# GitHubOfAndrew/TeAMOFlow

Hardware: AMD Instinct MI355X
Metric: train_interactions_per_sec (higher is better)
Workload: dtype f32

## Files before the change

include/tmf.h:

```cpp
#ifndef TMF_H
#define TMF_H

#include <stddef.h>
#include <stdint.h>

#ifdef __cplusplus
extern "C" {
#endif

#define TMF_VERSION 203

#define TMF_OK 0
#define TMF_E_INVALID (-1)
#define TMF_E_LAUNCH (-2)
#define TMF_E_UNSUPPORTED (-3)

#define TMF_EPI_ADAM 0
#define TMF_EPI_GRAD 1

int tmf_version(void);
const char* tmf_last_error(void);

int tmf_padded_ld(int n_components);

// ... 94 lines not shown
                         int n_components, void* stream);
int tmf_wmrb_scores3_bf16(const tmf_slice_lists* lists, const void* U, const void* V, float* sp, float* p,
                          int n_components, void* stream);
int tmf_wmrb_scores5_users_per_workgroup(void);
int tmf_wmrb_scores5_supported(int n_components, int bf16, int64_t n_items);
size_t tmf_wmrb_scores5_workspace_bytes(int64_t n_wg, int32_t n_windows, int wgs_per_launch);
int tmf_wmrb_scores5_f32(const int32_t* ids, const int32_t* outs, const int64_t* wg_ptr, int64_t n_wg, int64_t n_users,
                         int64_t n_items, const void* U, const void* V, float* sp, float* p, int n_components,
                         int wgs_per_launch, const int32_t* wstart, int32_t n_windows, int lag, void* workspace,
                         size_t workspace_bytes, void* stream);
int tmf_wmrb_scores5_bf16(const int32_t* ids, const int32_t* outs, const int64_t* wg_ptr, int64_t n_wg, int64_t n_users,
                          int64_t n_items, const void* U, const void* V, float* sp, float* p, int n_components,
                          int wgs_per_launch, const int32_t* wstart, int32_t n_windows, int lag, void* workspace,
                          size_t workspace_bytes, void* stream);
int tmf_wmrb_scores6_users_per_group(void);
int tmf_wmrb_scores6_supported(int n_components, int bf16, int64_t n_items);
int tmf_wmrb_scores6_f32(const int32_t* ids, const int32_t* outs, const int64_t* chunk_ptr, int64_t n_groups, int32_t n_slices,
                         int64_t n_users, int64_t n_items, const void* U, const void* V, float* sp, float* p, int n_components,
                         void* stream);
int tmf_wmrb_scores6_bf16(const int32_t* ids, const int32_t* outs, const int64_t* chunk_ptr, int64_t n_groups, int32_t n_slices,
                          int64_t n_users, int64_t n_items, const void* U, const void* V, float* sp, float* p, int n_components,
                          void* stream);
int tmf_wmrb_scores7_users_per_group(void);
int tmf_wmrb_scores7_slots(void);
int tmf_wmrb_scores7_supported(int n_components, int bf16, int64_t n_items);
int tmf_wmrb_scores7_f32(const void* steps, const int32_t* place, const int64_t* sub_step, const int64_t* sub_place,
                         const int32_t* chunk_sub, int64_t n_groups, int32_t n_slices, int64_t n_users, int64_t n_items,
                         const void* U, const void* V, float* sp, float* p, int n_components, void* stream);
int tmf_wmrb_hinge2(const int64_t* rowptr, const float* val, const float* p, const float* sp, int32_t n_users,
                    int32_t n_samples, float c, float* delta, float* D, float* loss_part, void* stream);
int tmf_wmrb_hinge2_ordered(const int64_t* rowptr, const float* val, const float* p, const float* sp, int32_t n_users,
                            int32_t n_samples, float c, float* delta, float* D, float* loss_part, const int32_t* user_order,
                            void* stream);
int tmf_bpr_pairs(const int64_t* rowptr, const float* val, const float* p, const float* sp, int32_t n_users, int32_t n_samples,
                  float* delta, float* D, float* loss_part, const int32_t* user_order, void* stream);
int tmf_warp_pairs(const int64_t* rowptr, const float* val, const float* p, const float* sp, int32_t n_users, int32_t n_samples,
                   int32_t n_items, float* delta, float* D, float* loss_part, const int32_t* user_order, void* stream);
int tmf_warp_pairs_ranked(const int64_t* rowptr, const float* val, const float* p, const float* sp, const uint16_t* rank,
                          int32_t n_users, int32_t n_samples, int32_t n_items, float* delta, float* D, float* loss_part,
                          const int32_t* user_order, void* stream);
int tmf_softmax_pairs(const int64_t* rowptr, const float* val, const float* p, const float* sp, int32_t n_users, int32_t n_samples,
                      float c, float* delta, float* D, float* loss_part, const int32_t* user_order, void* stream);
int tmf_wmrb_gradu3_f32(const tmf_slice_lists* lists, const float* D, const float* delta, const void* V, float* part,
                        int per_slice_launches, int n_components, void* stream);
int tmf_wmrb_gradu3_bf16(const tmf_slice_lists* lists, const float* D, const float* delta, const void* V, float* part,
                         int per_slice_launches, int n_components, void* stream);
// ... 194 lines not shown
```

teamoflow_amd/_engine.py:

```python
import ctypes
import os

import torch

from . import _lib

DEFAULT_CHUNK = 1024
PART_BUDGET = int(os.environ.get('TMF_PART_BUDGET', 8 << 30))


def row_bytes(n_components, dtype=torch.float32):
    return _lib.padded_ld(n_components, dtype) * (2 if dtype is torch.bfloat16 else 4)


def _excl_cumsum(x):
    out = torch.zeros(x.numel() + 1, dtype=torch.int64, device=x.device)
    torch.cumsum(x, 0, out=out[1:])
    return out


def take_interactions(indices, values, keep, user_offset=0, item_offset=0):
    u = indices[:, 0][keep] - user_offset
    j = indices[:, 1][keep] - item_offset
    return torch.stack([u, j], dim=1), values[keep]
# ... 486 lines not shown
            self.outs[q0:q0 + q.numel()] = torch.where(r < c, outs_sorted[src], torch.full_like(src, self.PAD).to(i32))
            del q, st, r, c, src
        self.n_entries, self.n_padded = E, E8
        return ptr8, rowptr


class Scores6Plan(_ScoreStreams):

    def __init__(self, plan, wplan, n_components, dtype=torch.float32, slice_bytes=None):
        lib = _lib.load_library()
        self.key = (int(n_components), dtype)
        UG = int(lib.tmf_wmrb_scores6_users_per_group())
        n = plan.n_items
        self.n_groups = ng = -(-wplan.R.shape[0] // UG)
        slice_bytes = int(os.environ.get('TMF_S6_SLICE_BYTES', slice_bytes or SCORES6_SLICE_BYTES))
        ns = int(min(max(1, -(-n * row_bytes(n_components, dtype) // slice_bytes)), max(1, (2 ** 31 - 1) // max(ng, 1))))
        width = -(-n // ns)
        self.n_slices = ns = -(-n // width)
        self.chunk_ptr, _ = self._build(plan, wplan, UG, lambda grp, item: (item // width) * ng + grp, ns * ng)


SCORES7_SLICE_BYTES = 4 << 20
SCORES7_MIN_SHARE = 1.5


def scores7_wanted(plan, wplan, n_components, dtype=torch.float32):
    env = os.environ.get('TMF_SCORES7')
    if env == '0' or wplan is None or not wplan.sliced or not plan.col_u.is_cuda:
        return False
    m, S = wplan.R.shape
    if m * S >= 2 ** 31 or plan.nnz >= 2 ** 31:
        return False
    lib = _lib.load_library()
    if not lib.tmf_wmrb_scores7_supported(int(n_components), int(dtype is torch.bfloat16), int(plan.n_items)):
        return False
    if env == '1':
        return True
    if os.environ.get('TMF_SCORES5') == '1' or os.environ.get('TMF_SCORES6') == '1':
        return False
    if plan.n_items * row_bytes(n_components, dtype) < 8 * VISIT_SLICE_BYTES:
        return False
    UG = int(lib.tmf_wmrb_scores7_users_per_group())
    return UG * (S + plan.nnz / max(m, 1)) / plan.n_items >= SCORES7_MIN_SHARE


class Scores7Plan:

    K = 4

    def __init__(self, plan, wplan, n_components, dtype=torch.float32, slice_bytes=None, slots=None):
        lib = _lib.load_library()
        self.key = (int(n_components), dtype)
        dev, i32, i64, K = plan.col_u.device, torch.int32, torch.int64, self.K
        self.users_per_group = UG = int(lib.tmf_wmrb_scores7_users_per_group())
        self.pad_slot = cap = int(lib.tmf_wmrb_scores7_slots())
        self.slots = SL = max(1, min(cap, int(os.environ.get('TMF_S7_SLOTS', slots or cap))))
        m, S = wplan.R.shape
        n, nnz = plan.n_items, plan.nnz
        E = nnz + m * S
        self.n_groups = ng = -(-m // UG)
        slice_bytes = int(os.environ.get('TMF_S7_SLICE_BYTES', slice_bytes or SCORES7_SLICE_BYTES))
        ns = int(min(max(1, -(-n * row_bytes(n_components, dtype) // slice_bytes)), max(1, (2 ** 31 - 1) // max(ng, 1))))
        self.width = width = -(-n // ns)
        self.n_slices = ns = -(-n // width)
        nc = ns * ng
        ar = torch.arange(E, device=dev, dtype=i64)
# ... 39 lines not shown
        self.sub_step = _excl_cumsum(sub_steps)
        del subA, sub_steps, run_steps
        pos = ar - run_start[run_of]
        del ar, run_start
        stepA = run_step0[run_of] + pos // K
        k = pos % K
        del pos, run_of, run_step0
        users = torch.zeros(n_steps, K, dtype=i64, device=dev)
        slot4 = torch.full((n_steps, K), cap, dtype=i64, device=dev)
        first = k == 0
        users[stepA[first]] = luA[first].to(i64)[:, None]
        users[stepA, k] = luA.to(i64)
        slot4[stepA, k] = slotA.to(i64)
        steps = torch.zeros(n_steps + 1, 4, dtype=i32, device=dev)
        steps[stepA[first], 0] = itemA[first]
        del first, stepA, k, luA, slotA, itemA
        w = users[:, 0] | (users[:, 1] << 8) | (users[:, 2] << 16) | (users[:, 3] << 24)
        steps[:n_steps, 1] = torch.where(w >= 2 ** 31, w - 2 ** 32, w).to(i32)
        steps[:n_steps, 2] = (slot4[:, 0] | (slot4[:, 1] << 16)).to(i32)
        steps[:n_steps, 3] = (slot4[:, 2] | (slot4[:, 3] << 16)).to(i32)
        self.steps = steps
        self.n_entries = E


def scores5_wanted(plan, wplan, n_components, dtype=torch.float32):
    if os.environ.get('TMF_SCORES5') != '1' or wplan is None or not wplan.sliced or not plan.col_u.is_cuda:
        return False
    m, S = wplan.R.shape
    if m * S >= 2 ** 31 or plan.nnz >= 2 ** 31:
        return False
    return bool(_lib.load_library().tmf_wmrb_scores5_supported(int(n_components), int(dtype is torch.bfloat16), int(plan.n_items)))


class Scores5Plan(_ScoreStreams):

    def __init__(self, plan, wplan, n_components, dtype=torch.float32, slice_bytes=None):
        lib = _lib.load_library()
        dev = plan.col_u.device
        self.key = (int(n_components), dtype)
        UB = int(lib.tmf_wmrb_scores5_users_per_workgroup())
        n = plan.n_items
        self.n_wg = n_wg = -(-wplan.R.shape[0] // UB)
        slice_bytes = int(os.environ.get('TMF_S5_SLICE_BYTES', slice_bytes or (512 << 10)))
        ns = int(min(max(1, -(-n * row_bytes(n_components, dtype) // slice_bytes)), 4096, max(1, (2 ** 31 - 1) // max(n_wg, 1))))
        width = -(-n // ns)
        self.n_slices = ns
# ... 78 lines not shown

    def _adopt_wplan(self):
        plan, wplan, dtype, dev = self.plan, self.wplan, self.dtype, self.plan.col_u.device
        need = dict(slab=max(self._slab_fixed,
                             (wplan.seg_e.n_slab if wplan is not None and wplan.seg_e is not None else 0) * self.ld,
                             (wplan.vrows.n_slab if wplan is not None and wplan.vrows is not None else 0) * self.ld))
        self.row_stationary = False
        if wplan is not None and wplan.sliced:
            m, S = wplan.R.shape
            self.row_stationary = row_stationary_wanted(m, plan.n_items, S, plan.nnz, self.r, dtype)
            self.users_per_launch = int(os.environ.get('TMF_G4_USERS', 32768))
            if self.row_stationary:
                nb = _lib.load_library().tmf_wmrb_gradu4_workspace_bytes(m, wplan.n_slices, self.users_per_launch)
                self.g4_sync = torch.zeros(max(nb // 4, 1), dtype=torch.int32, device=dev)
            ns = wplan.n_slices
            if ns * m * self.ld * 4 <= PART_BUDGET:
                self.part_layers, self.gradu_launches = ns, 0
            elif wplan.xcd_major:
                self.part_layers, self.gradu_launches = min(8, ns), 3
            else:
                self.part_layers, self.gradu_launches = 1, 1
            need.update(sp=m * S, pk=max(plan.nnz, 1), part=self.part_layers * max(m, 1) * self.ld)
            if scores7_wanted(plan, wplan, self.r, dtype):
                if wplan.s7 is None or wplan.s7.key != (self.r, dtype):
                    if os.environ.get('TMF_SCORES7') == '1':
                        wplan.s7 = Scores7Plan(plan, wplan, self.r, dtype)
                    else:
                        try:
                            wplan.s7 = Scores7Plan(plan, wplan, self.r, dtype)
                        except torch.OutOfMemoryError:
                            wplan.s7 = None
            else:
                wplan.s7 = None
            if wplan.s7 is None and scores6_wanted(plan, wplan, self.r, dtype):
                if wplan.s6 is None or wplan.s6.key != (self.r, dtype):
                    wplan.s6 = Scores6Plan(plan, wplan, self.r, dtype)
            else:
                wplan.s6 = None
            if wplan.seg_e is not None and scores5_wanted(plan, wplan, self.r, dtype):
                if wplan.s5 is None or wplan.s5.key != (self.r, dtype):
                    wplan.s5 = Scores5Plan(plan, wplan, self.r, dtype)
            else:
                wplan.s5 = None
        if wplan is not None and wplan.rows4:
            L = _lib.load_library()
            per_group = L.tmf_wsum_rows4_rows_per_group(self.r, int(dtype is torch.bfloat16))
            if not per_group:
                raise ValueError('the row-stationary item pass needs rows of at least 16 lanes')
            cus = torch.cuda.get_device_properties(dev).multi_processor_count if torch.cuda.is_available() else 256
            self.rows4_per_launch = int(os.environ.get('TMF_ROWS4_PER_LAUNCH', 2 * cus * per_group))
            n_work = wplan.vrows.n_vrows if wplan.vrows is not None else plan.n_items
            nb = L.tmf_wsum_rows4_workspace_bytes(n_work, wplan.user_chunks, self.rows4_per_launch)
            self.rows4_sync = torch.zeros(max(nb // 4, 1), dtype=torch.int32, device=dev)
        return need
# ... 387 lines not shown

def epoch_logistic(st, adam, loss_out, weighted=False, item_epi=_lib.EPI_ADAM, item_out=None, prof=None, user_epi=_lib.EPI_ADAM,
                   user_out=None):
    _list_passes(st, adam, 'tmf_logistic_pass', 'logistic', st.loss_part, None, (int(bool(weighted)),), loss_out, item_epi, item_out,
                 prof, user_epi, user_out)


def epoch_kl(st, adam, loss_out, item_epi=_lib.EPI_ADAM, item_out=None, prof=None, user_epi=_lib.EPI_ADAM, user_out=None):
    lib, p, r = _lib.get(), st.plan, st.r
    s = _lib.stream_ptr()
    _timed(prof, 'kl_moments', lambda: getattr(lib, 'tmf_kl_moments' + st.sfx)(
        p.seg_u.cstruct(), _lib.ptr(p.col_u), _lib.ptr(p.val_u), _lib.ptr(st.U), _lib.ptr(st.V), _lib.ptr(st.kl_part), r, s))
    _timed(prof, 'kl_coeffs', lambda: lib.tmf_kl_coeffs(_lib.ptr(st.kl_part), p.seg_u.nseg, _lib.ptr(loss_out), _lib.ptr(st.kl_coef), s))
    _list_passes(st, adam, 'tmf_kl_pass', 'kl', st.kl_coef, st.kl_coef, (), None, item_epi, item_out, prof, user_epi, user_out)


def _wmrb_user_pass_sliced(lib, st, adam, c, prof=None, user_epi=_lib.EPI_ADAM, U_out=None, pairs='hinge'):
    p, w, r = st.plan, st.wplan, st.r
    i32 = ctypes.c_int32
    m, S, ns = p.n_users, w.S, w.n_slices
    s = _lib.stream_ptr()
    lists = w.lists(p)
    s5, s6, s7 = w.s5, w.s6, w.s7
    if s7 is not None:
        _timed(prof, 'wmrb_scores', lambda: lib.tmf_wmrb_scores7_f32(
            _lib.ptr(s7.steps), _lib.ptr(s7.place), _lib.ptr(s7.sub_step), _lib.ptr(s7.sub_place), _lib.ptr(s7.chunk_sub), s7.n_groups,
            i32(s7.n_slices), m, p.n_items, _lib.ptr(st.U), _lib.ptr(st.V), _lib.ptr(st.sp), _lib.ptr(st.pk), r, s))
    elif s6 is not None:
        _timed(prof, 'wmrb_scores', lambda: getattr(lib, 'tmf_wmrb_scores6' + st.sfx)(
            _lib.ptr(s6.ids), _lib.ptr(s6.outs), _lib.ptr(s6.chunk_ptr), s6.n_groups, i32(s6.n_slices), m, p.n_items, _lib.ptr(st.U),
            _lib.ptr(st.V), _lib.ptr(st.sp), _lib.ptr(st.pk), r, s))
    elif s5 is not None:
        _timed(prof, 'wmrb_scores', lambda: getattr(lib, 'tmf_wmrb_scores5' + st.sfx)(
            _lib.ptr(s5.ids), _lib.ptr(s5.outs), _lib.ptr(s5.wg_ptr), s5.n_wg, m, p.n_items, _lib.ptr(st.U), _lib.ptr(st.V),
            _lib.ptr(st.sp), _lib.ptr(st.pk), r, s5.wgs_per_launch, _lib.ptr(s5.wstart) if s5.paced else None, i32(s5.n_windows),
            s5.lag, _lib.ptr(s5.sync) if s5.paced else None, s5.sync.numel() * 4, s))
    else:
        _timed(prof, 'wmrb_scores', lambda: getattr(lib, 'tmf_wmrb_scores3' + st.sfx)(lists, _lib.ptr(st.U), _lib.ptr(st.V), _lib.ptr(st.sp),
                                                                                _lib.ptr(st.pk), r, s))
    if pairs == 'bpr':
        _timed(prof, 'bpr_pairs', lambda: lib.tmf_bpr_pairs(_lib.ptr(p.rowptr_u), _lib.ptr(p.val_u), _lib.ptr(st.pk), _lib.ptr(st.sp),
                                                            i32(m), i32(S), _lib.ptr(w.delta), _lib.ptr(w.D), _lib.ptr(st.loss_part),
                                                            _lib.ptr(w.hinge_order), s))
    elif pairs == 'warp':
        rank = w.sample_rank()
        _timed(prof, 'warp_pairs', lambda: lib.tmf_warp_pairs_ranked(_lib.ptr(p.rowptr_u), _lib.ptr(p.val_u), _lib.ptr(st.pk),
                                                                     _lib.ptr(st.sp), _lib.ptr(rank), i32(m), i32(S), i32(p.n_items),
# ... 63 lines not shown
```

teamoflow_amd/_lib.py:

```python
import ctypes
import os
import subprocess

import torch

_HERE = os.path.dirname(os.path.abspath(__file__))
LIB_PATH = os.environ.get('TMF_LIB', os.path.join(_HERE, 'libtmf.so'))
CSRC = os.path.join(_HERE, 'csrc')

EPI_ADAM, EPI_GRAD = 0, 1


class EngineUnavailable(RuntimeError):
    pass


class EngineError(RuntimeError):
    pass


class Adam(ctypes.Structure):
    _fields_ = [('alpha', ctypes.c_float), ('one_minus_b1', ctypes.c_float), ('one_minus_b2', ctypes.c_float),
                ('eps', ctypes.c_float)]

# ... 47 lines not shown
    'tmf_mse_pass_f32': (_I, [_SEG, _P, _P, _P, _P, _P, _P, _P, _I, _I, Adam, _P]),
    'tmf_kl_moments_f32': (_I, [_SEG, _P, _P, _P, _P, _P, _I, _P]),
    'tmf_kl_moments_bf16': (_I, [_SEG, _P, _P, _P, _P, _P, _I, _P]),
    'tmf_kl_coeffs': (_I, [_P, _L, _P, _P, _P]),
    'tmf_kl_pass_f32': (_I, [_SEG, _P, _P, _P, _P, _P, _P, _P, _I, _I, Adam, _P]),
    'tmf_kl_pass_bf16': (_I, [_SEG, _P, _P, _P, _P, _P, _P, _P, _I, _I, Adam, _P]),
    'tmf_logistic_pass_f32': (_I, [_SEG, _P, _P, _P, _P, _P, _P, _P, _I, _I, Adam, _I, _P]),
    'tmf_logistic_pass_bf16': (_I, [_SEG, _P, _P, _P, _P, _P, _P, _P, _I, _I, Adam, _I, _P]),
    'tmf_wsum_pass_f32': (_I, [_SEG, _P, _P, _P, _P, _P, _P, _P, _I, _I, Adam, _P]),
    'tmf_wsum_rows4_rows_per_group': (_I, [_I, _I]),
    'tmf_wsum_rows4_workspace_bytes': (_SZ, [_I32, _I32, _I32]),
    'tmf_wsum_rows4_f32': (_I, [_P, _I32, _I32, _P, _P, _P, _P, _P, _P, _I, _I, Adam, _I32, _P, _SZ, _P]),
    'tmf_wsum_rows5_workspace_bytes': (_SZ, [_I32, _I32, _I32]),
    'tmf_wsum_rows5_f32': (_I, [_P, _I32, _I32, _P, _P, _P, _P, _P, _P, _P, _P, _P, _P, _P, _I32, _I, _I, Adam, _I32, _P, _SZ, _P]),
    'tmf_combine_rows_f32': (_I, [_P, _P, _L, _P, _P, _P, _I, _I, Adam, _P]),
    'tmf_wmrb_user_pass_f32': (_I, [_P, _P, _P, _P, _I32, _I32, _F, _P, _P, _P, _P, _P, _P, _P, _I, _I, Adam, _P]),
    'tmf_wmrb_user_pass_fits': (_I, [_I32, _I]),
    'tmf_wmrb_scores3_f32': (_I, [_SL, _P, _P, _P, _P, _I, _P]),
    'tmf_wmrb_scores6_users_per_group': (_I, []),
    'tmf_wmrb_scores6_supported': (_I, [_I, _I, _L]),
    'tmf_wmrb_scores6_f32': (_I, [_P, _P, _P, _L, _I32, _L, _L, _P, _P, _P, _P, _I, _P]),
    'tmf_wmrb_scores7_users_per_group': (_I, []),
    'tmf_wmrb_scores7_slots': (_I, []),
    'tmf_wmrb_scores7_supported': (_I, [_I, _I, _L]),
    'tmf_wmrb_scores7_f32': (_I, [_P, _P, _P, _P, _P, _L, _I32, _L, _L, _P, _P, _P, _P, _I, _P]),
    'tmf_wmrb_scores5_users_per_workgroup': (_I, []),
    'tmf_wmrb_scores5_supported': (_I, [_I, _I, _L]),
    'tmf_wmrb_scores5_workspace_bytes': (_SZ, [_L, _I32, _I]),
    'tmf_wmrb_scores5_f32': (_I, [_P, _P, _P, _L, _L, _L, _P, _P, _P, _P, _I, _I, _P, _I32, _I, _P, _SZ, _P]),
    'tmf_wmrb_hinge2': (_I, [_P, _P, _P, _P, _I32, _I32, _F, _P, _P, _P, _P]),
    'tmf_wmrb_hinge2_ordered': (_I, [_P, _P, _P, _P, _I32, _I32, _F, _P, _P, _P, _P, _P]),
    'tmf_bpr_pairs': (_I, [_P, _P, _P, _P, _I32, _I32, _P, _P, _P, _P, _P]),
    'tmf_warp_pairs': (_I, [_P, _P, _P, _P, _I32, _I32, _I32, _P, _P, _P, _P, _P]),
    'tmf_warp_pairs_ranked': (_I, [_P, _P, _P, _P, _P, _I32, _I32, _I32, _P, _P, _P, _P, _P]),
    'tmf_softmax_pairs': (_I, [_P, _P, _P, _P, _I32, _I32, _F, _P, _P, _P, _P, _P]),
    'tmf_wmrb_gradu3_f32': (_I, [_SL, _P, _P, _P, _P, _I, _I, _P]),
    'tmf_wmrb_gradu4_supported': (_I, [_I, _I]),
    'tmf_wmrb_gradu4_workspace_bytes': (_SZ, [_I32, _I32, _I32]),
    'tmf_wmrb_gradu4_f32': (_I, [_SL, _P, _P, _P, _P, _P, _I, _I, Adam, _I32, _P, _SZ, _P]),
    'tmf_wmrb_finish_f32': (_I, [_P, _I32, _I32, _P, _P, _I, _I, Adam, _P]),
    'tmf_adam_fresh_rows_f32': (_I, [_P, _P, _L, _I, Adam, _P]),
    'tmf_bias_colsum_part_rows': (_L, [_L]),
    'tmf_bias_colsum_f32': (_I, [_P, _L, _I, _P, _L, _P, _P]),
    'tmf_bias_adam_f32': (_I, [_P, _L, _P, _P, _I, Adam, _P]),
    'tmf_adam_bias_rows_f32': (_I, [_P, _P, _P, _P, _L, _I, Adam, _P]),
    'tmf_feat_pass_f32': (_I, [_SEG, _P, _P, _P, _P, _P, _P, _I, _I, Adam, _P]),
# ... 146 lines not shown
```

teamoflow_amd/csrc/tmf_wmrb.hip:

```cpp
#include <math.h>
#include <stdlib.h>

#include <type_traits>

#include "tmf_common.h"

namespace tmf {

constexpr int kThreads = 256;
constexpr int kWaves = kThreads / 64;
constexpr int kPosChunk = 512;
constexpr int kUnrollW = 4;
constexpr int kG4Unroll = 4;

__host__ __device__ inline int round4(int x) { return (x + 3) & ~3; }

__host__ __device__ inline int sp_padded(int S) {
    const int nf4 = (S + 3) / 4;
    const int per = ((nf4 + 2 * kWaves - 1) / (2 * kWaves) + 1) & ~1;
    return 4 * 2 * kWaves * per;
}

__device__ __forceinline__ void count_ge0_x4(int& c0, int& c1, float x0, float x1, float x2, float x3) {
    unsigned long long m0, m1, m2, m3;
// ... 1259 lines not shown
        }                                                                                                                   \
    }
        TMF_DISPATCH(T, geom, CALL);
#undef CALL
    }
    return check_launch("tmf_wmrb_scores6");
}

namespace tmf {
constexpr int kS7Users = 256;
constexpr int kS7Slots = 6144;
constexpr int kS7K = 4;
constexpr int kS7Waves = 16;
constexpr int kS7Flight = 2;
constexpr uint32_t kS7RowBytes = 512;
constexpr size_t kS7Lds = (size_t)kS7Users * kS7RowBytes + (size_t)(kS7Slots + 64) * sizeof(float);

struct S7Streams {
    const int4* steps;
    const int32_t* place;
    const int64_t* sub_step;
    const int64_t* sub_place;
    const int32_t* chunk_sub;
};

__global__ __launch_bounds__(64 * kS7Waves) void k_wmrb_scores7(S7Streams a, int64_t chunk0, int64_t n_groups, int64_t n_users,
                                                                const float* __restrict__ U, const float* __restrict__ V,
                                                                float* __restrict__ sp, float* __restrict__ p) {
    constexpr int NG = 8 * kS7Waves, NT = 64 * kS7Waves, FL = kS7Flight;
    extern __shared__ __attribute__((aligned(16))) char smem_raw[];
    float* sbuf = reinterpret_cast<float*>(smem_raw + (size_t)kS7Users * kS7RowBytes);
    const int tid = threadIdx.x, lane = tid & 63, g = lane & 7, gid = tid >> 3;
    const int64_t chunk = chunk0 + blockIdx.x;
    const int sub_b = a.chunk_sub[chunk], sub_e = a.chunk_sub[chunk + 1];
    if (sub_b == sub_e) return;
    const int64_t ubeg = (chunk % n_groups) * kS7Users;
    const int nu = (int)((n_users - ubeg < kS7Users) ? n_users - ubeg : kS7Users);
    {
        const tmf_f4* src = reinterpret_cast<const tmf_f4*>(reinterpret_cast<const char*>(U) + ubeg * (int64_t)kS7RowBytes);
        tmf_f4* dst = reinterpret_cast<tmf_f4*>(smem_raw);
        for (int i = tid; i < nu * (int)(kS7RowBytes / 16); i += NT) dst[i] = __builtin_nontemporal_load(src + i);
    }
    __syncthreads();
    const uint32_t par = (lane >> 4) & 1;
    const uint32_t offA = 16u * g + 128u * par, offB = 16u * g + 128u * (par ^ 1u);
    struct Row {
        float4 v[4];
    };
    auto dot = [](const Row& x, const Row& y) {
        float q[4];
#pragma unroll
        for (int v = 0; v < 4; ++v) {
            tmf_f2 a = tmf_f2{x.v[v].x, x.v[v].y} * tmf_f2{y.v[v].x, y.v[v].y};
            a = __builtin_elementwise_fma(tmf_f2{x.v[v].z, x.v[v].w}, tmf_f2{y.v[v].z, y.v[v].w}, a);
            q[v] = a.x + a.y;
        }
        return (q[0] + q[2]) + (q[1] + q[3]);
    };
    for (int sub = sub_b; sub < sub_e; ++sub) {
        const int64_t st0 = a.sub_step[sub];
        const int nsteps = (int)(a.sub_step[sub + 1] - st0);
        const int64_t pl0 = a.sub_place[sub];
        const int nslots = (int)(a.sub_place[sub + 1] - pl0);
        const int4* rec0 = a.steps + st0;
        const int mine = nsteps > gid ? (nsteps - gid + NG - 1) / NG : 0;
        const int rounds = __builtin_amdgcn_readfirstlane(mine);
        const int32_t* pl = a.place + pl0;
        int32_t where[kS7Slots / NT];
#pragma unroll
        for (int q = 0; q < kS7Slots / NT; ++q) where[q] = (tid + NT * q < nslots) ? __builtin_nontemporal_load(pl + tid + NT * q) : 0;
        if (rounds > 0) {
            auto fetch = [&](int i) {
                const int st = gid + NG * i;
                return rec0[st < nsteps ? st : nsteps - 1];
            };
            auto gather = [&](Row& y, const int4& r) {
                const char* base = reinterpret_cast<const char*>(V);
                const uint32_t oa = row_byte_off<kS7RowBytes>((uint32_t)r.x, offA), ob = row_byte_off<kS7RowBytes>((uint32_t)r.x, offB);
                y.v[0] = *reinterpret_cast<const float4*>(base + oa);
                y.v[1] = *reinterpret_cast<const float4*>(base + ob);
                y.v[2] = *reinterpret_cast<const float4*>(base + oa + 256);
                y.v[3] = *reinterpret_cast<const float4*>(base + ob + 256);
            };
            auto finish = [&](const Row& y, const int4& r, int i) {
                float s[kS7K];
#pragma unroll
                for (int k = 0; k < kS7K; ++k) {
                    const uint32_t lu = ((uint32_t)r.y >> (8 * k)) & 0xffu;
                    const char* xa = smem_raw + (lu * kS7RowBytes + offA);
                    const char* xb = smem_raw + (lu * kS7RowBytes + offB);
                    Row x;
                    x.v[0] = *reinterpret_cast<const float4*>(xa);
                    x.v[1] = *reinterpret_cast<const float4*>(xb);
                    x.v[2] = *reinterpret_cast<const float4*>(xa + 256);
                    x.v[3] = *reinterpret_cast<const float4*>(xb + 256);
                    float t = dot(x, y);
                    t += TMF_DPP_MOV(t, 0xB1);
                    t += TMF_DPP_MOV(t, 0x4E);
                    t += TMF_DPP_MOV(t, 0x141);
                    s[k] = t;
                }
                const float mine_s = (g & 2) ? ((g & 1) ? s[3] : s[2]) : ((g & 1) ? s[1] : s[0]);
                const uint32_t w = (g & 2) ? (uint32_t)r.w : (uint32_t)r.z;
                uint32_t slot = (g & 1) ? (w >> 16) : (w & 0xffffu);
                slot = (slot < (uint32_t)kS7Slots && gid + NG * i < nsteps) ? slot : (uint32_t)kS7Slots;
                if (g < kS7K) sbuf[slot] = mine_s;
            };
            Row y[FL];
            int4 rec[2 * FL];
#pragma unroll
            for (int j = 0; j < FL; ++j) rec[j] = fetch(j);
#pragma unroll
            for (int j = 0; j < FL; ++j) {
                gather(y[j], rec[j]);
                rec[FL + j] = fetch(FL + j);
            }
            int i = 0;
            for (; i + 2 * FL <= rounds; i += 2 * FL) {
#pragma unroll
                for (int j = 0; j < 2 * FL; ++j) {
                    __builtin_amdgcn_sched_barrier(0);
                    finish(y[j % FL], rec[j], i + j);
                    __builtin_amdgcn_sched_barrier(0);
                    gather(y[j % FL], rec[(j + FL) % (2 * FL)]);
                    rec[j] = fetch(i + j + 2 * FL);
                }
            }
            const int rem = rounds - i;
#pragma unroll
            for (int j = 0; j < 2 * FL - 1; ++j) {
                if (j < rem) {
                    __builtin_amdgcn_sched_barrier(0);
                    finish(y[j % FL], rec[j], i + j);
                    __builtin_amdgcn_sched_barrier(0);
                    if (j + FL < rem) gather(y[j % FL], rec[j + FL]);
                }
            }
        }
        __syncthreads();
#pragma unroll
        for (int q = 0; q < kS7Slots / NT; ++q)
            if (tid + NT * q < nslots)
                __builtin_nontemporal_store(sbuf[tid + NT * q], where[q] >= 0 ? sp + where[q] : p + ~where[q]);
        __syncthreads();
    }
}

}

static bool s7_supported(int n_components, int bf16, int64_t n_items) {
    return !bf16 && n_components >= 65 && n_components <= 128 && s6_supported(n_components, 0, n_items);
}

static int wmrb_scores7_impl(const void* steps, const int32_t* place, const int64_t* sub_step, const int64_t* sub_place,
                             const int32_t* chunk_sub, int64_t n_groups, int32_t n_slices, int64_t n_users, int64_t n_items,
                             const void* U, const void* V, float* sp, float* p, int n_components, void* stream) {
    if (n_users == 0 || n_slices == 0) return TMF_OK;
    TMF_REQUIRE(steps && place && sub_step && sub_place && chunk_sub && U && V && sp && p, "wmrb_scores7: null pointer");
    TMF_REQUIRE(n_groups == (n_users + kS7Users - 1) / kS7Users && n_slices > 0, "wmrb_scores7: %lld groups for %lld users (%d per group), %d slices",
                (long long)n_groups, (long long)n_users, kS7Users, n_slices);
    if (!s7_supported(n_components, 0, n_items)) {
        set_error("wmrb_scores7: needs fp32 rows of 65..128 components and fewer than 2^24 items in a table below 4 GB "
                  "(got %d components, %lld items)", n_components, (long long)n_items);
        return TMF_E_UNSUPPORTED;
    }
    static LdsGrant grant;
    if (int rc = grant_dynamic_lds(reinterpret_cast<const void*>(&k_wmrb_scores7), kS7Lds, grant)) return rc;
    const S7Streams a{static_cast<const int4*>(steps), place, sub_step, sub_place, chunk_sub};
    const int64_t per_slice = n_groups * 64 * kS7Waves;
    const int max_slices = (int)((((int64_t)1 << 32) - 1) / per_slice);
    TMF_REQUIRE(max_slices >= 1, "wmrb_scores7: %lld user groups exceed one launch", (long long)n_groups);
    for (int s0 = 0; s0 < n_slices; s0 += max_slices) {
        const int nsl = (n_slices - s0 < max_slices) ? n_slices - s0 : max_slices;
        hipLaunchKernelGGL(k_wmrb_scores7, dim3((unsigned)(n_groups * nsl)), dim3(64 * kS7Waves), kS7Lds, (hipStream_t)stream, a,
                           (int64_t)s0 * n_groups, n_groups, n_users, (const float*)U, (const float*)V, sp, p);
    }
    return check_launch("tmf_wmrb_scores7");
}

static int s5_launches(int64_t n_wg, int wgs_per_launch) { return (int)((n_wg + wgs_per_launch - 1) / wgs_per_launch); }
static int s5_wgs_per_launch(int wgs_per_launch) {
    if (wgs_per_launch > 0) return wgs_per_launch;
    int dev = 0, cus = 256;
    if (hipGetDevice(&dev) == hipSuccess) (void)hipDeviceGetAttribute(&cus, hipDeviceAttributeMultiprocessorCount, dev);
    return cus > 0 ? cus : 256;
}

template <typename T>
static int wmrb_scores5_impl(const int32_t* ids, const int32_t* outs, const int64_t* wg_ptr, int64_t n_wg, int64_t n_users,
                             int64_t n_items, const void* U, const void* V, float* sp, float* p, int n_components,
                             int wgs_per_launch, const int32_t* wstart, int32_t n_windows, int lag, void* workspace,
// ... 85 lines not shown
                                         const void* V, float* part, int per_slice_launches, int n_components,            \
                                         void* stream) {                                                                  \
        return wmrb_gradu3_impl<T_>(lists, D, delta, V, part, per_slice_launches, n_components, stream);                  \
    }                                                                                                                     \
    extern "C" int tmf_wmrb_gradu4_##SFX(const tmf_slice_lists* lists, const float* D, const float* delta, const void* V,  \
                                         const void* U_old, void* U_out, int n_components, int epi, tmf_adam adam,       \
                                         int32_t users_per_launch, void* workspace, size_t workspace_bytes, void* stream) { \
        return wmrb_gradu4_impl<T_>(lists, D, delta, V, U_old, U_out, n_components, epi, adam, users_per_launch, workspace, \
                                    workspace_bytes, stream);                                                            \
    }                                                                                                                     \
    extern "C" int tmf_wmrb_finish_##SFX(const float* part, int32_t n_slices, int32_t n_users, const void* U_old,         \
                                         void* U_out, int n_components, int epi, tmf_adam adam, void* stream) {           \
        return wmrb_finish_impl<T_>(part, n_slices, n_users, U_old, U_out, n_components, epi, adam, stream);               \
    }

TMF_SLICED_ENTRY_POINTS(f32, float)
TMF_SLICED_ENTRY_POINTS(bf16, __bf16)

extern "C" int tmf_wmrb_scores6_users_per_group(void) { return tmf::kS6Users; }
extern "C" int tmf_wmrb_scores6_supported(int n_components, int bf16, int64_t n_items) { return s6_supported(n_components, bf16, n_items); }
extern "C" int tmf_wmrb_scores7_f32(const void* steps, const int32_t* place, const int64_t* sub_step, const int64_t* sub_place,
                                    const int32_t* chunk_sub, int64_t n_groups, int32_t n_slices, int64_t n_users, int64_t n_items,
                                    const void* U, const void* V, float* sp, float* p, int n_components, void* stream) {
    return wmrb_scores7_impl(steps, place, sub_step, sub_place, chunk_sub, n_groups, n_slices, n_users, n_items, U, V, sp, p,
                             n_components, stream);
}
extern "C" int tmf_wmrb_scores7_users_per_group(void) { return tmf::kS7Users; }
extern "C" int tmf_wmrb_scores7_slots(void) { return tmf::kS7Slots; }
extern "C" int tmf_wmrb_scores7_supported(int n_components, int bf16, int64_t n_items) { return s7_supported(n_components, bf16, n_items); }
extern "C" int tmf_wmrb_scores5_users_per_workgroup(void) { return tmf::kS5Users; }
extern "C" size_t tmf_wmrb_scores5_workspace_bytes(int64_t n_wg, int32_t n_windows, int wgs_per_launch) {
    if (n_wg <= 0 || n_windows <= 1) return 0;
    return (size_t)s5_launches(n_wg, s5_wgs_per_launch(wgs_per_launch)) * 8 * (size_t)n_windows * tmf::kS5Stride * sizeof(int);
}
extern "C" int tmf_wmrb_scores5_supported(int n_components, int bf16, int64_t n_items) {
    const tmf::RowGeom geom = bf16 ? tmf::row_geom_bf16(n_components) : tmf::row_geom(n_components);
    const int64_t row_bytes = (int64_t)geom.ld * (bf16 ? 2 : 4);
    return geom.G == 32 && row_bytes * tmf::kS5Users <= 128 * 1024 && n_items > 0 && n_items < (1 << 24) &&
           n_items * row_bytes < ((int64_t)1 << 32);
}
```

Baseline: 1.261 billion.

## Sort scores7 steps by slot fill and balance waves by cost

Adds a plan-time pass that sorts each sub-block's step records by how many of their K user slots are filled. It also computes per-wave step ranges from a cost model so that each wave gets a similar share of work. The kernel then runs FILL-specialised variants (4, 3, 2, 1) that skip dot products for empty slots and no longer use the gid-strided assignment. This removes wasted LDS reads and FMAs on padded slots and evens out load across waves, at the cost of extra preprocessing memory and more code paths. The variant is on by default.

After: 1.301 billion, median of 6. 1.03x the previous value.

```diff
diff --git a/include/tmf.h b/include/tmf.h
--- a/include/tmf.h
+++ b/include/tmf.h
@@ -140,6 +140,11 @@
                           int64_t n_users, int64_t n_items, const void* U, const void* V, float* sp, float* p, int n_components,
                           void* stream);
 int tmf_wmrb_scores7_users_per_group(void);
+int tmf_wmrb_scores7_waves(void);
+int tmf_wmrb_scores7_fill_f32(const void* steps, const int32_t* place, const int64_t* sub_step, const int64_t* sub_place,
+                              const int32_t* chunk_sub, const int32_t* sub_wave, const int32_t* sub_fill, int64_t n_groups,
+                              int32_t n_slices, int64_t n_users, int64_t n_items, const void* U, const void* V, float* sp, float* p,
+                              int n_components, void* stream);
 int tmf_wmrb_scores7_slots(void);
 int tmf_wmrb_scores7_supported(int n_components, int bf16, int64_t n_items);
 int tmf_wmrb_scores7_f32(const void* steps, const int32_t* place, const int64_t* sub_step, const int64_t* sub_place,
diff --git a/teamoflow_amd/_engine.py b/teamoflow_amd/_engine.py
--- a/teamoflow_amd/_engine.py
+++ b/teamoflow_amd/_engine.py
@@ -532,6 +532,8 @@
 
 SCORES7_SLICE_BYTES = 4 << 20
 SCORES7_MIN_SHARE = 1.5
+SCORES7_COST_STEP, SCORES7_COST_SLOT = 3, 2
+SCORES7_FILL = True
 
 
 def scores7_wanted(plan, wplan, n_components, dtype=torch.float32):
@@ -552,6 +554,10 @@
         return False
     UG = int(lib.tmf_wmrb_scores7_users_per_group())
     return UG * (S + plan.nnz / max(m, 1)) / plan.n_items >= SCORES7_MIN_SHARE
+
+
+def scores7_fill_wanted():
+    return os.environ.get('TMF_S7_FILL', '1' if SCORES7_FILL else '0') != '0'
 
 
 class Scores7Plan:
@@ -637,6 +643,45 @@
         self.steps = steps
         self.n_entries = E
 
+    sub_wave = sub_fill = None
+
+    def order_by_fill(self):
+        if self.sub_wave is not None:
+            return self
+        W = int(_lib.load_library().tmf_wmrb_scores7_waves())
+        K, cap, n_steps, n_sub = self.K, self.pad_slot, self.n_steps, self.n_sub
+        dev, i32, i64 = self.steps.device, torch.int32, torch.int64
+        rec = self.steps[:n_steps]
+        fill = torch.zeros(n_steps, dtype=i64, device=dev)
+        for word in (rec[:, 2], rec[:, 3]):
+            fill += ((word & 0xffff) != cap).to(i64) + (((word >> 16) & 0xffff) != cap).to(i64)
+        sub_of = torch.zeros(n_steps, dtype=i64, device=dev)
+        if n_sub > 1:
+            sub_of.scatter_add_(0, self.sub_step[1:n_sub], torch.ones(n_sub - 1, dtype=i64, device=dev))
+        sub_of = torch.cumsum(sub_of, 0)
+        key = sub_of * K + (K - fill)
+        del fill, sub_of
+        order = torch.sort(key, stable=True)[1]
+        cnt = torch.bincount(key, minlength=K * n_sub).view(n_sub, K)
+        del key
+        steps = torch.zeros_like(self.steps)
+        old64, new64 = self.steps.view(i64), steps.view(i64)
+        for half in range(2):
+            new64[:n_steps, half] = old64[:n_steps, half][order]
+        del order, rec, old64, new64
+        self.steps = steps
+        self.sub_fill = cnt.to(i32).contiguous()
+        zero = torch.zeros(n_sub, 1, dtype=i64, device=dev)
+        slope = torch.tensor([SCORES7_COST_STEP + SCORES7_COST_SLOT * f for f in range(K, 0, -1)], dtype=i64, device=dev)
+        step_edge = torch.cat([zero, torch.cumsum(cnt, 1)], 1)
+        cost_edge = torch.cat([zero, torch.cumsum(cnt * slope, 1)], 1) * W
+        target = cost_edge[:, K:] // W * torch.arange(1, W, device=dev, dtype=i64)
+        cls = (target[:, :, None] >= cost_edge[:, None, 1:K]).sum(2)
+        cut = torch.gather(step_edge, 1, cls) + (target - torch.gather(cost_edge, 1, cls)) // (W * slope[cls])
+        cut = torch.minimum((cut + 4) // 8 * 8, step_edge[:, K:])
+        self.sub_wave = torch.cat([zero, cut, step_edge[:, K:]], 1).to(i32).contiguous()
+        return self
+
 
 def scores5_wanted(plan, wplan, n_components, dtype=torch.float32):
     if os.environ.get('TMF_SCORES5') != '1' or wplan is None or not wplan.sliced or not plan.col_u.is_cuda:
@@ -761,14 +806,15 @@
                 self.part_layers, self.gradu_launches = 1, 1
             need.update(sp=m * S, pk=max(plan.nnz, 1), part=self.part_layers * max(m, 1) * self.ld)
             if scores7_wanted(plan, wplan, self.r, dtype):
-                if wplan.s7 is None or wplan.s7.key != (self.r, dtype):
+                try:
+                    if wplan.s7 is None or wplan.s7.key != (self.r, dtype):
+                        wplan.s7 = Scores7Plan(plan, wplan, self.r, dtype)
+                    if scores7_fill_wanted():
+                        wplan.s7.order_by_fill()
+                except torch.OutOfMemoryError:
                     if os.environ.get('TMF_SCORES7') == '1':
-                        wplan.s7 = Scores7Plan(plan, wplan, self.r, dtype)
-                    else:
-                        try:
-                            wplan.s7 = Scores7Plan(plan, wplan, self.r, dtype)
-                        except torch.OutOfMemoryError:
-                            wplan.s7 = None
+                        raise
+                    wplan.s7 = None
             else:
                 wplan.s7 = None
             if wplan.s7 is None and scores6_wanted(plan, wplan, self.r, dtype):
@@ -1202,7 +1248,12 @@
     s = _lib.stream_ptr()
     lists = w.lists(p)
     s5, s6, s7 = w.s5, w.s6, w.s7
-    if s7 is not None:
+    if s7 is not None and s7.sub_wave is not None:
+        _timed(prof, 'wmrb_scores', lambda: lib.tmf_wmrb_scores7_fill_f32(
+            _lib.ptr(s7.steps), _lib.ptr(s7.place), _lib.ptr(s7.sub_step), _lib.ptr(s7.sub_place), _lib.ptr(s7.chunk_sub),
+            _lib.ptr(s7.sub_wave), _lib.ptr(s7.sub_fill), s7.n_groups, i32(s7.n_slices), m, p.n_items, _lib.ptr(st.U), _lib.ptr(st.V),
+            _lib.ptr(st.sp), _lib.ptr(st.pk), r, s))
+    elif s7 is not None:
         _timed(prof, 'wmrb_scores', lambda: lib.tmf_wmrb_scores7_f32(
             _lib.ptr(s7.steps), _lib.ptr(s7.place), _lib.ptr(s7.sub_step), _lib.ptr(s7.sub_place), _lib.ptr(s7.chunk_sub), s7.n_groups,
             i32(s7.n_slices), m, p.n_items, _lib.ptr(st.U), _lib.ptr(st.V), _lib.ptr(st.sp), _lib.ptr(st.pk), r, s))
diff --git a/teamoflow_amd/_lib.py b/teamoflow_amd/_lib.py
--- a/teamoflow_amd/_lib.py
+++ b/teamoflow_amd/_lib.py
@@ -93,6 +93,8 @@
     'tmf_wmrb_scores6_f32': (_I, [_P, _P, _P, _L, _I32, _L, _L, _P, _P, _P, _P, _I, _P]),
     'tmf_wmrb_scores7_users_per_group': (_I, []),
     'tmf_wmrb_scores7_slots': (_I, []),
+    'tmf_wmrb_scores7_waves': (_I, []),
+    'tmf_wmrb_scores7_fill_f32': (_I, [_P, _P, _P, _P, _P, _P, _P, _L, _I32, _L, _L, _P, _P, _P, _P, _I, _P]),
     'tmf_wmrb_scores7_supported': (_I, [_I, _I, _L]),
     'tmf_wmrb_scores7_f32': (_I, [_P, _P, _P, _P, _P, _L, _I32, _L, _L, _P, _P, _P, _P, _I, _P]),
     'tmf_wmrb_scores5_users_per_workgroup': (_I, []),
diff --git a/teamoflow_amd/csrc/tmf_wmrb.hip b/teamoflow_amd/csrc/tmf_wmrb.hip
--- a/teamoflow_amd/csrc/tmf_wmrb.hip
+++ b/teamoflow_amd/csrc/tmf_wmrb.hip
@@ -1305,6 +1305,8 @@
     const int64_t* sub_step;
     const int64_t* sub_place;
     const int32_t* chunk_sub;
+    const int32_t* sub_wave;
+    const int32_t* sub_fill;
 };
 
 __global__ __launch_bounds__(64 * kS7Waves) void k_wmrb_scores7(S7Streams a, int64_t chunk0, int64_t n_groups, int64_t n_users,
@@ -1327,6 +1329,7 @@
     __syncthreads();
     const uint32_t par = (lane >> 4) & 1;
     const uint32_t offA = 16u * g + 128u * par, offB = 16u * g + 128u * (par ^ 1u);
+    const uint32_t slot_sel = 0x0c0c0000u | ((2u * (g & 3) + 1u) << 8) | (2u * (g & 3));
     struct Row {
         float4 v[4];
     };
@@ -1340,85 +1343,108 @@
         }
         return (q[0] + q[2]) + (q[1] + q[3]);
     };
+    auto run = [&](auto fill_tag, const int4* rec0, int first, int stride, int end, int rounds) {
+        constexpr int FILL = decltype(fill_tag)::value;
+        auto fetch = [&](int i) {
+            const int st = first + stride * i;
+            return rec0[st < end ? st : end - 1];
+        };
+        auto gather = [&](Row& y, const int4& r) {
+            const char* base = reinterpret_cast<const char*>(V);
+            const uint32_t oa = row_byte_off<kS7RowBytes>((uint32_t)r.x, offA), ob = row_byte_off<kS7RowBytes>((uint32_t)r.x, offB);
+            y.v[0] = *reinterpret_cast<const float4*>(base + oa);
+            y.v[1] = *reinterpret_cast<const float4*>(base + ob);
+            y.v[2] = *reinterpret_cast<const float4*>(base + oa + 256);
+            y.v[3] = *reinterpret_cast<const float4*>(base + ob + 256);
+        };
+        auto finish = [&](const Row& y, const int4& r, int i) {
+            float s[FILL];
+#pragma unroll
+            for (int k = 0; k < FILL; ++k) {
+                const uint32_t lu = ((uint32_t)r.y >> (8 * k)) & 0xffu;
+                const char* xa = smem_raw + (lu * kS7RowBytes + offA);
+                const char* xb = smem_raw + (lu * kS7RowBytes + offB);
+                Row x;
+                x.v[0] = *reinterpret_cast<const float4*>(xa);
+                x.v[1] = *reinterpret_cast<const float4*>(xb);
+                x.v[2] = *reinterpret_cast<const float4*>(xa + 256);
+                x.v[3] = *reinterpret_cast<const float4*>(xb + 256);
+                float t = dot(x, y);
+                t += TMF_DPP_MOV(t, 0xB1);
+                t += TMF_DPP_MOV(t, 0x4E);
+                t += TMF_DPP_MOV(t, 0x141);
+                s[k] = t;
+            }
+            float mine_s = s[0];
+            if constexpr (FILL == 2) mine_s = (g & 1) ? s[1] : s[0];
+            if constexpr (FILL == 3) mine_s = (g & 2) ? s[2] : ((g & 1) ? s[1] : s[0]);
+            if constexpr (FILL == 4) mine_s = (g & 2) ? ((g & 1) ? s[3] : s[2]) : ((g & 1) ? s[1] : s[0]);
+            uint32_t slot = __builtin_amdgcn_perm((uint32_t)r.w, (uint32_t)r.z, slot_sel);
+            slot = (slot < (uint32_t)kS7Slots && first + stride * i < end) ? slot : (uint32_t)kS7Slots;
+            if (g < FILL) sbuf[slot] = mine_s;
+        };
+        Row y[FL];
+        int4 rec[2 * FL];
+#pragma unroll
+        for (int j = 0; j < FL; ++j) rec[j] = fetch(j);
+#pragma unroll
+        for (int j = 0; j < FL; ++j) {
+            gather(y[j], rec[j]);
+            rec[FL + j] = fetch(FL + j);
+        }
+        int i = 0;
+        for (; i + 2 * FL <= rounds; i += 2 * FL) {
+#pragma unroll
+            for (int j = 0; j < 2 * FL; ++j) {
+                __builtin_amdgcn_sched_barrier(0);
+                finish(y[j % FL], rec[j], i + j);
+                __builtin_amdgcn_sched_barrier(0);
+                gather(y[j % FL], rec[(j + FL) % (2 * FL)]);
+                rec[j] = fetch(i + j + 2 * FL);
+            }
+        }
+        const int rem = rounds - i;
+#pragma unroll
+        for (int j = 0; j < 2 * FL - 1; ++j) {
+            if (j < rem) {
+                __builtin_amdgcn_sched_barrier(0);
+                finish(y[j % FL], rec[j], i + j);
+                __builtin_amdgcn_sched_barrier(0);
+                if (j + FL < rem) gather(y[j % FL], rec[j + FL]);
+            }
+        }
+    };
+    const int wave = __builtin_amdgcn_readfirstlane(tid >> 6);
+    const bool by_fill = a.sub_wave != nullptr;
     for (int sub = sub_b; sub < sub_e; ++sub) {
         const int64_t st0 = a.sub_step[sub];
         const int nsteps = (int)(a.sub_step[sub + 1] - st0);
         const int64_t pl0 = a.sub_place[sub];
         const int nslots = (int)(a.sub_place[sub + 1] - pl0);
         const int4* rec0 = a.steps + st0;
-        const int mine = nsteps > gid ? (nsteps - gid + NG - 1) / NG : 0;
-        const int rounds = __builtin_amdgcn_readfirstlane(mine);
         const int32_t* pl = a.place + pl0;
         int32_t where[kS7Slots / NT];
 #pragma unroll
         for (int q = 0; q < kS7Slots / NT; ++q) where[q] = (tid + NT * q < nslots) ? __builtin_nontemporal_load(pl + tid + NT * q) : 0;
-        if (rounds > 0) {
-            auto fetch = [&](int i) {
-                const int st = gid + NG * i;
-                return rec0[st < nsteps ? st : nsteps - 1];
-            };
-            auto gather = [&](Row& y, const int4& r) {
-                const char* base = reinterpret_cast<const char*>(V);
-                const uint32_t oa = row_byte_off<kS7RowBytes>((uint32_t)r.x, offA), ob = row_byte_off<kS7RowBytes>((uint32_t)r.x, offB);
-                y.v[0] = *reinterpret_cast<const float4*>(base + oa);
-                y.v[1] = *reinterpret_cast<const float4*>(base + ob);
-                y.v[2] = *reinterpret_cast<const float4*>(base + oa + 256);
-                y.v[3] = *reinterpret_cast<const float4*>(base + ob + 256);
-            };
-            auto finish = [&](const Row& y, const int4& r, int i) {
-                float s[kS7K];
-#pragma unroll
-                for (int k = 0; k < kS7K; ++k) {
-                    const uint32_t lu = ((uint32_t)r.y >> (8 * k)) & 0xffu;
-                    const char* xa = smem_raw + (lu * kS7RowBytes + offA);
-                    const char* xb = smem_raw + (lu * kS7RowBytes + offB);
-                    Row x;
-                    x.v[0] = *reinterpret_cast<const float4*>(xa);
-                    x.v[1] = *reinterpret_cast<const float4*>(xb);
-                    x.v[2] = *reinterpret_cast<const float4*>(xa + 256);
-                    x.v[3] = *reinterpret_cast<const float4*>(xb + 256);
-                    float t = dot(x, y);
-                    t += TMF_DPP_MOV(t, 0xB1);
-                    t += TMF_DPP_MOV(t, 0x4E);
-                    t += TMF_DPP_MOV(t, 0x141);
-                    s[k] = t;
-                }
-                const float mine_s = (g & 2) ? ((g & 1) ? s[3] : s[2]) : ((g & 1) ? s[1] : s[0]);
-                const uint32_t w = (g & 2) ? (uint32_t)r.w : (uint32_t)r.z;
-                uint32_t slot = (g & 1) ? (w >> 16) : (w & 0xffffu);
-                slot = (slot < (uint32_t)kS7Slots && gid + NG * i < nsteps) ? slot : (uint32_t)kS7Slots;
-                if (g < kS7K) sbuf[slot] = mine_s;
-            };
-            Row y[FL];
-            int4 rec[2 * FL];
-#pragma unroll
-            for (int j = 0; j < FL; ++j) rec[j] = fetch(j);
-#pragma unroll
-            for (int j = 0; j < FL; ++j) {
-                gather(y[j], rec[j]);
-                rec[FL + j] = fetch(FL + j);
-            }
-            int i = 0;
-            for (; i + 2 * FL <= rounds; i += 2 * FL) {
-#pragma unroll
-                for (int j = 0; j < 2 * FL; ++j) {
-                    __builtin_amdgcn_sched_barrier(0);
-                    finish(y[j % FL], rec[j], i + j);
-                    __builtin_amdgcn_sched_barrier(0);
-                    gather(y[j % FL], rec[(j + FL) % (2 * FL)]);
-                    rec[j] = fetch(i + j + 2 * FL);
-                }
-            }
-            const int rem = rounds - i;
-#pragma unroll
-            for (int j = 0; j < 2 * FL - 1; ++j) {
-                if (j < rem) {
-                    __builtin_amdgcn_sched_barrier(0);
-                    finish(y[j % FL], rec[j], i + j);
-                    __builtin_amdgcn_sched_barrier(0);
-                    if (j + FL < rem) gather(y[j % FL], rec[j + FL]);
-                }
-            }
+        int lo = 8 * wave, hi = nsteps, stride = NG, wb = 0, we = 0, cls = 0;
+        if (by_fill) {
+            const int32_t* sw = a.sub_wave + (int64_t)sub * (kS7Waves + 1) + wave;
+            wb = __builtin_amdgcn_readfirstlane(sw[0]);
+            we = __builtin_amdgcn_readfirstlane(sw[1]);
+            cls = __builtin_amdgcn_readfirstlane(a.sub_fill[(int64_t)sub * kS7K]);
+            lo = wb, hi = we < cls ? we : cls, stride = 8;
+        }
+        if (lo < hi) run(std::integral_constant<int, 4>{}, rec0, lo + (by_fill ? (gid & 7) : gid - 8 * wave), stride, hi, (hi - lo + stride - 1) / stride);
+        if (by_fill) {
+            const int32_t* sf = a.sub_fill + (int64_t)sub * kS7K;
+            int end = cls + __builtin_amdgcn_readfirstlane(sf[1]);
+            lo = wb > cls ? wb : cls, hi = we < end ? we : end, cls = end;
+            if (lo < hi) run(std::integral_constant<int, 3>{}, rec0, lo + (gid & 7), 8, hi, (hi - lo + 7) / 8);
+            end = cls + __builtin_amdgcn_readfirstlane(sf[2]);
+            lo = wb > cls ? wb : cls, hi = we < end ? we : end, cls = end;
+            if (lo < hi) run(std::integral_constant<int, 2>{}, rec0, lo + (gid & 7), 8, hi, (hi - lo + 7) / 8);
+            lo = wb > cls ? wb : cls, hi = we;
+            if (lo < hi) run(std::integral_constant<int, 1>{}, rec0, lo + (gid & 7), 8, hi, (hi - lo + 7) / 8);
         }
         __syncthreads();
 #pragma unroll
@@ -1436,10 +1462,11 @@
 }
 
 static int wmrb_scores7_impl(const void* steps, const int32_t* place, const int64_t* sub_step, const int64_t* sub_place,
-                             const int32_t* chunk_sub, int64_t n_groups, int32_t n_slices, int64_t n_users, int64_t n_items,
+                             const int32_t* chunk_sub, const int32_t* sub_wave, const int32_t* sub_fill, int64_t n_groups, int32_t n_slices, int64_t n_users, int64_t n_items,
                              const void* U, const void* V, float* sp, float* p, int n_components, void* stream) {
     if (n_users == 0 || n_slices == 0) return TMF_OK;
     TMF_REQUIRE(steps && place && sub_step && sub_place && chunk_sub && U && V && sp && p, "wmrb_scores7: null pointer");
+    TMF_REQUIRE(!sub_wave == !sub_fill, "wmrb_scores7: sub_wave and sub_fill come together");
     TMF_REQUIRE(n_groups == (n_users + kS7Users - 1) / kS7Users && n_slices > 0, "wmrb_scores7: %lld groups for %lld users (%d per group), %d slices",
                 (long long)n_groups, (long long)n_users, kS7Users, n_slices);
     if (!s7_supported(n_components, 0, n_items)) {
@@ -1449,7 +1476,7 @@
     }
     static LdsGrant grant;
     if (int rc = grant_dynamic_lds(reinterpret_cast<const void*>(&k_wmrb_scores7), kS7Lds, grant)) return rc;
-    const S7Streams a{static_cast<const int4*>(steps), place, sub_step, sub_place, chunk_sub};
+    const S7Streams a{static_cast<const int4*>(steps), place, sub_step, sub_place, chunk_sub, sub_wave, sub_fill};
     const int64_t per_slice = n_groups * 64 * kS7Waves;
     const int max_slices = (int)((((int64_t)1 << 32) - 1) / per_slice);
     TMF_REQUIRE(max_slices >= 1, "wmrb_scores7: %lld user groups exceed one launch", (long long)n_groups);
@@ -1581,9 +1608,18 @@
 extern "C" int tmf_wmrb_scores7_f32(const void* steps, const int32_t* place, const int64_t* sub_step, const int64_t* sub_place,
                                     const int32_t* chunk_sub, int64_t n_groups, int32_t n_slices, int64_t n_users, int64_t n_items,
                                     const void* U, const void* V, float* sp, float* p, int n_components, void* stream) {
-    return wmrb_scores7_impl(steps, place, sub_step, sub_place, chunk_sub, n_groups, n_slices, n_users, n_items, U, V, sp, p,
+    return wmrb_scores7_impl(steps, place, sub_step, sub_place, chunk_sub, nullptr, nullptr, n_groups, n_slices, n_users, n_items, U, V, sp, p,
                              n_components, stream);
 }
+extern "C" int tmf_wmrb_scores7_fill_f32(const void* steps, const int32_t* place, const int64_t* sub_step, const int64_t* sub_place,
+                                         const int32_t* chunk_sub, const int32_t* sub_wave, const int32_t* sub_fill, int64_t n_groups,
+                                         int32_t n_slices, int64_t n_users, int64_t n_items, const void* U, const void* V, float* sp,
+                                         float* p, int n_components, void* stream) {
+    TMF_REQUIRE(sub_wave && sub_fill, "wmrb_scores7_fill: null pointer");
+    return wmrb_scores7_impl(steps, place, sub_step, sub_place, chunk_sub, sub_wave, sub_fill, n_groups, n_slices, n_users, n_items, U, V,
+                             sp, p, n_components, stream);
+}
+extern "C" int tmf_wmrb_scores7_waves(void) { return tmf::kS7Waves; }
 extern "C" int tmf_wmrb_scores7_users_per_group(void) { return tmf::kS7Users; }
 extern "C" int tmf_wmrb_scores7_slots(void) { return tmf::kS7Slots; }
 extern "C" int tmf_wmrb_scores7_supported(int n_components, int bf16, int64_t n_items) { return s7_supported(n_components, bf16, n_items); }
```
